# loganmcbroom/Flan

Hardware: AMD Instinct MI355X
Metric: PV analysis+resynthesis frames/sec (2048-win, hop 512, 48 kHz) at 1/2/4/8 GPU (higher is better)
Workload: dtype f32; 1 GPU; 8 ch x 60 s x 48 kHz uniform noise per GPU, convert_to_PV(2048,512,dft 2048) -> convert_to_audio round trip; channels_per_gpu=8, parallelism=channel-shard x1

## Files before the change

flan_amd/csrc/conversions.hip:

```cpp
#include "flanhip_internal.h"
#include <atomic>
#include <memory>
#include "pv_kernels.h"
#include "pv_kernels_fast.h"
#include <type_traits>
#include "pv_kernels_v2.h"
#include "pv_kernels_v3.h"
#include "pv_kernels_eo.h"
#include "pv_kernels_any.h"
#include "pv_kernels_mr.h"
#include "pv_kernels_bs.h"
#include "pv_kernels_big.h"
#include "team_launch.h"
#include "sub_launch.h"
#include <algorithm>
#include <cstdlib>

namespace flanhip {


static constexpr size_t kMaxLds = 160 * 1024;

static constexpr int kMaxAnyDft = 1 << 20;
static bool fft_size( int dft ) { return is_pow2( dft ) && dft >= 32 && dft <= 8192; }
// ... 138 lines not shown
	return size_t( C ) * 8 + size_t( wpad ) * 4 + size_t( chains ) * ( size_t( padded_len( C + 1 ) ) * 8 + size_t( wpad ) * 4 );
	}

template<int LOG2C, int WAVES, int T = 1>
static int run_analyze( const AnalyzeParams & p, hipStream_t s )
	{
	const size_t lds = analyze_lds_bytes( 1 << LOG2C, p.window_size, WAVES, LOG2C >= 12 && T == 1 );
	FLANHIP_REQUIRE( lds <= kMaxLds, FLANHIP_ERR_UNSUPPORTED, "window/dft too large for LDS" );
	auto kern = k_analyze<LOG2C, WAVES, T>;
	FLANHIP_CHECK( hipFuncSetAttribute( reinterpret_cast<const void*>( kern ), hipFuncAttributeMaxDynamicSharedMemorySize, int( lds ) ) );
	const int64_t chains = int64_t( p.chains_per_channel ) * p.num_channels;
	const int64_t blocks = ( chains + WAVES - 1 ) / WAVES;
	FLANHIP_REQUIRE( blocks < ( int64_t( 1 ) << 31 ), FLANHIP_ERR_UNSUPPORTED, "too many chains for one launch" );
	hipLaunchKernelGGL( kern, dim3( (unsigned) blocks ), dim3( 64 * WAVES * T ), lds, s, p );
	FLANHIP_CHECK( hipGetLastError() );
	return FLANHIP_OK;
	}

#define FLANHIP_V3_CFGS_9( X ) X( 0, 8, 4, 4, 1 )
#define FLANHIP_V3_CFGS_8( X ) X( 0, 4, 3, 4, 1 )
struct V3Cfg { int waves, occ, nv; };
static V3Cfg v3_cfg( int dft )
	{
	const int v = debug_options().ana_variant;
#define X( I, W, O, N, P ) if( v == I ) return V3Cfg{ W, O, N };
	if( dft == 1024 ) { FLANHIP_V3_CFGS_9( X ) return V3Cfg{ 8, 4, 4 }; }
	FLANHIP_V3_CFGS_8( X )
#undef X
	return V3Cfg{ 4, 3, 4 };
	}
static int v3_index( int dft )
	{
	const int v = debug_options().ana_variant;
#define X( I, W, O, N, P ) if( v == I ) return I;
	if( dft == 1024 ) { FLANHIP_V3_CFGS_9( X ) return 0; }
	FLANHIP_V3_CFGS_8( X )
#undef X
	return 0;
	}
static bool v3_size( int dft ) { return dft == 1024 || dft == 512; }
static int group_size_of( int dft ) { return dft == 2048 ? 8 : dft == 4096 ? 4 : v3_size( dft ) ? v3_cfg( dft ).waves : 8; }
static constexpr int kTeamWaves12 = 8;
static int generic_target_chains( int dft ) { const int cus = cu_count(); return dft >= 8192 ? cus : dft == 4096 ? 2 * cus : dft == 2048 ? 4 * cus : 16 * cus; }
static int fast_target_chains( int dft, bool synth )
	{
	if( const int v = debug_options().target_chains ) { if( v > 0 ) return v; }
	return cu_count() * ( dft == 4096 ? 4 : dft == 2048 ? 8 : 4 * v3_cfg( dft ).occ );
	}

template<int WAVES, bool SUMS, int NV, int ABL = 0>
static int run_analyze_v2( const AnalyzeParams & p, const FastTables & tb, hipStream_t s )
	{
	FLANHIP_REQUIRE( ( int64_t( WAVES ) * p.L + 2 ) * std::max( int64_t( p.hop ) * 4, int64_t( 8200 ) ) < ( int64_t( 1 ) << 32 ), FLANHIP_ERR_UNSUPPORTED, "chain length x hop too large for the dft 2048 kernel" );
	const size_t lds = V2Lds::bytes( WAVES );
	static_assert( V2Lds::bytes( WAVES ) <= kMaxLds, "LDS budget" );
	auto kern = k_analyze_v2<WAVES, SUMS, NV, ABL>;
	FLANHIP_CHECK( hipFuncSetAttribute( reinterpret_cast<const void*>( kern ), hipFuncAttributeMaxDynamicSharedMemorySize, int( lds ) ) );
	const int64_t blocks = int64_t( ( p.chains_per_channel + WAVES - 1 ) / WAVES ) * p.num_channels;
	FLANHIP_REQUIRE( blocks < ( int64_t( 1 ) << 31 ), FLANHIP_ERR_UNSUPPORTED, "too many chains for one launch" );
	hipLaunchKernelGGL( kern, dim3( (unsigned) blocks ), dim3( 64 * WAVES ), lds, s, p, tb );
	FLANHIP_CHECK( hipGetLastError() );
	return FLANHIP_OK;
	}

template<bool SUMS>
static int run_analyze_v2_variant( int v, const AnalyzeParams & p, const FastTables & tb, hipStream_t s )
	{
	switch( v )
		{
		default: return run_analyze_v2<8, SUMS, 8>( p, tb, s );
#ifdef FLANHIP_ABLATIONS
		case 101: return run_analyze_v2<8, SUMS, 8, 1>( p, tb, s );
		case 102: return run_analyze_v2<8, SUMS, 8, 2>( p, tb, s );
		case 104: return run_analyze_v2<8, SUMS, 8, 4>( p, tb, s );
		case 108: return run_analyze_v2<8, SUMS, 8, 8>( p, tb, s );
		case 116: return run_analyze_v2<8, SUMS, 8, 16>( p, tb, s );
		case 132: return run_analyze_v2<8, SUMS, 8, 32>( p, tb, s );
		case 106: return run_analyze_v2<8, SUMS, 8, 6>( p, tb, s );
		case 124: return run_analyze_v2<8, SUMS, 8, 24>( p, tb, s );
		case 163: return run_analyze_v2<8, SUMS, 8, 63>( p, tb, s );
		case 164: return run_analyze_v2<8, SUMS, 8, 64>( p, tb, s );
		case 228: return run_analyze_v2<8, SUMS, 8, 128>( p, tb, s );
		case 292: return run_analyze_v2<8, SUMS, 8, 192>( p, tb, s );
		case 139: return run_analyze_v2<8, SUMS, 8, 39>( p, tb, s );
		case 107: return run_analyze_v2<8, SUMS, 8, 7>( p, tb, s );
		case 356: return run_analyze_v2<8, SUMS, 8, 256>( p, tb, s );
		case 1124: return run_analyze_v2<8, SUMS, 8, 1024>( p, tb, s );
		case 1163: return run_analyze_v2<8, SUMS, 8, 1024 + 39>( p, tb, s );
		case 612: return run_analyze_v2<8, SUMS, 8, 512>( p, tb, s );
		case 868: return run_analyze_v2<8, SUMS, 8, 768>( p, tb, s );
#endif
		}
	}

template<int LOG2C, bool SUMS, int WAVES, int OCC, int NV, int PF>
static int run_analyze_v3( const AnalyzeParams & p, hipStream_t s )
	{
	using L = V3Lds<LOG2C>;
	FLANHIP_REQUIRE( ( int64_t( WAVES ) * p.L + 2 ) * std::max( int64_t( p.hop ) * 4, int64_t( ( L::C + 1 ) * 8 ) ) < ( int64_t( 1 ) << 32 ), FLANHIP_ERR_UNSUPPORTED, "chain length x hop too large for the dft 1024 / 512 kernel" );
	const size_t lds = L::bytes( WAVES, true );
	static_assert( L::bytes( WAVES, true ) * ( 4 * OCC / WAVES ) <= kMaxLds, "LDS budget" );
	auto kern = k_analyze_v3<LOG2C, WAVES, SUMS, OCC, NV, ( PF & 255 ), ( PF >> 8 )>;
	FLANHIP_CHECK( hipFuncSetAttribute( reinterpret_cast<const void*>( kern ), hipFuncAttributeMaxDynamicSharedMemorySize, int( lds ) ) );
	const int64_t blocks = int64_t( ( p.chains_per_channel + WAVES - 1 ) / WAVES ) * p.num_channels;
	FLANHIP_REQUIRE( blocks < ( int64_t( 1 ) << 31 ), FLANHIP_ERR_UNSUPPORTED, "too many chains for one launch" );
	hipLaunchKernelGGL( kern, dim3( (unsigned) blocks ), dim3( 64 * WAVES ), lds, s, p );
	FLANHIP_CHECK( hipGetLastError() );
	return FLANHIP_OK;
	}
template<bool SUMS>
static int run_analyze_v3_cfg( int dft, const AnalyzeParams & p, hipStream_t s )
	{
	const int idx = v3_index( dft );
#define X( I, W, O, N, P ) if( idx == I ) return run_analyze_v3<9, SUMS, W, O, N, P>( p, s );
	if( dft == 1024 ) { FLANHIP_V3_CFGS_9( X ) }
#undef X
#define X( I, W, O, N, P ) if( idx == I ) return run_analyze_v3<8, SUMS, W, O, N, P>( p, s );
	if( dft == 512 ) { FLANHIP_V3_CFGS_8( X ) }
#undef X
	return FLANHIP_ERR_UNSUPPORTED;
// ... 707 lines not shown

int flanhip_synthesize_dev_fused_checked( const flanhip_MF * d_pv, int64_t ch, int64_t F, int bins, float sr, float ar, int W,
	float * d_out, void * d_ws, int * d_nan, void * stream )
	{
	return launch_synthesize( d_pv, ch, F, bins, sr, ar, W, d_out, d_ws, d_nan, 2, (hipStream_t) stream );
	}

int flanhip_analyze( const float * audio, int64_t ch, int64_t n, float sr, int W, int hop, int dft,
	flanhip_MF * out, int64_t * num_pv_frames, volatile int * cancel )
	{
	FLANHIP_REQUIRE( audio && out, FLANHIP_ERR_INVALID_ARG, "null buffer" );
	FLANHIP_REQUIRE( ch > 0 && n >= 0 && hop >= 1, FLANHIP_ERR_INVALID_ARG, "bad sizes" );
	if( int rc = require_device() ) return rc;
	const int64_t F = n / hop + 1;
	const int bins = dft / 2 + 1;
	if( num_pv_frames ) *num_pv_frames = F;
	if( cancelled( cancel ) ) return FLANHIP_ERR_CANCELLED;
	DeviceBuffer d_audio, d_pv;
	if( int rc = d_audio.alloc( sizeof( float ) * size_t( ch ) * n ) ) return rc;
	if( int rc = d_pv.alloc( sizeof( flanhip_MF ) * size_t( ch ) * F * bins ) ) return rc;
	if( int rc_t = flanhip_upload( d_audio.p, audio, sizeof( float ) * size_t( ch ) * n ) ) return rc_t;
	if( cancelled( cancel ) ) return FLANHIP_ERR_CANCELLED;
	if( int rc = launch_analyze( (const float*) d_audio.p, ch, n, sr, W, hop, dft, (flanhip_MF*) d_pv.p, nullptr, nullptr ) ) return rc;
	if( int rc = wait_cancellable( nullptr, cancel ? poll_volatile_int : nullptr, const_cast<int*>( cancel ) ) ) return rc;
	if( int rc_t = flanhip_download( out, d_pv.p, sizeof( flanhip_MF ) * size_t( ch ) * F * bins ) ) return rc_t;
	return FLANHIP_OK;
	}

int flanhip_synthesize_dev_stages( const flanhip_MF * d_pv, int64_t ch, int64_t F, int bins, float sr, float ar, int W,
	float * d_out, void * d_ws, int * d_nan, int presummed, int stages, void * stream )
	{
	FLANHIP_REQUIRE( presummed >= 0 && presummed <= 2, FLANHIP_ERR_INVALID_ARG, "presummed: 0, 1 or 2" );
	return launch_synthesize( d_pv, ch, F, bins, sr, ar, W, d_out, d_ws, d_nan, presummed, (hipStream_t) stream, nullptr, nullptr, false, stages );
	}

void flanhip_debug_option( int which, int value )
	{
	DebugOptions & o = debug_options();
	switch( which )
		{
		case FLANHIP_DEBUG_CHAIN_LEN:       o.chain_len = value; break;
		case FLANHIP_DEBUG_TARGET_CHAINS:   o.target_chains = value; break;
		case FLANHIP_DEBUG_FORCE_GENERIC:   o.force_generic = value; break;
		case FLANHIP_DEBUG_NO_FAST_DIV:     o.no_fast_div = value; break;
		case FLANHIP_DEBUG_ANA_VARIANT:     o.ana_variant = value; break;
		case FLANHIP_DEBUG_SYN_VARIANT:     o.syn_variant = value; break;
		case FLANHIP_DEBUG_ANA4096_OLD:     o.ana11_old = value; break;
		case FLANHIP_DEBUG_SYN4096_OLD:     o.syn11_old = value; break;
		case FLANHIP_DEBUG_RESAMPLE_DIRECT: o.resample_direct = value; break;
		case FLANHIP_DEBUG_FORCE_DIRECT:    o.force_direct = value; break;
		case FLANHIP_DEBUG_INLINE_FIXUP:    o.inline_fixup = value; break;
		case FLANHIP_DEBUG_WIDE_OFFSETS:    o.wide_offsets = value; break;
		case FLANHIP_DEBUG_NO_SUB:          o.no_sub = value; break;
		default: break;
		}
	}
#ifdef FLANHIP_STAMPS
int flanhip_debug_read_stamps( unsigned long long * out16 )
	{
	FLANHIP_CHECK( hipDeviceSynchronize() );
	FLANHIP_CHECK( hipMemcpyFromSymbol( out16, HIP_SYMBOL( g_stamp_acc ), 16 * sizeof( unsigned long long ) ) );
	unsigned long long zero[16] = { 0 };
	FLANHIP_CHECK( hipMemcpyToSymbol( HIP_SYMBOL( g_stamp_acc ), zero, sizeof( zero ) ) );
	return FLANHIP_OK;
	}
int flanhip_debug_read_spans( unsigned long long * out8192 )
	{
	FLANHIP_CHECK( hipDeviceSynchronize() );
	FLANHIP_CHECK( hipMemcpyFromSymbol( out8192, HIP_SYMBOL( g_stamp_span ), 8192 * sizeof( unsigned long long ) ) );
	return FLANHIP_OK;
	}
#endif

size_t flanhip_synthesize_workspace_bytes( int64_t ch, int64_t F, int bins, float sr, float ar, int W )
	{
	SynthLayout lay;
	if( synth_layout( ch, F, bins, sr, ar, W, &lay ) ) return 0;
	size_t bytes = lay.total_bytes;
	if( v3_size( lay.dft ) )
		{
		DebugOptions & o = debug_options();
		const int keep = o.ana_variant;
		for( int v = 0; v < 3; ++v )
			{
			o.ana_variant = v;
			SynthLayout alt;
			if( !synth_layout( ch, F, bins, sr, ar, W, &alt ) ) bytes = std::max( bytes, alt.total_bytes );
			}
		o.ana_variant = keep;
		}
	return bytes;
	}

int flanhip_synthesize_dev( const flanhip_MF * d_pv, int64_t ch, int64_t F, int bins, float sr, float ar, int W,
	float * d_out, void * d_ws, int * d_nan, void * stream )
	{
	return launch_synthesize( d_pv, ch, F, bins, sr, ar, W, d_out, d_ws, d_nan, false, (hipStream_t) stream );
	}

int flanhip_synthesize( const flanhip_MF * pv, int64_t ch, int64_t F, int bins, float sr, float ar, int W,
	float * out, int * nan_flag, volatile int * cancel )
	{
	FLANHIP_REQUIRE( pv && out, FLANHIP_ERR_INVALID_ARG, "null buffer" );
	SynthLayout lay;
	if( int rc = synth_layout( ch, F, bins, sr, ar, W, &lay ) ) return rc;
	if( int rc = require_device() ) return rc;
// ... 22 lines not shown
```

flan_amd/csrc/flanhip_internal.h:

```cpp
#pragma once
#include <hip/hip_runtime.h>
#include <cstdarg>
#include <cstdint>
#include <cstdio>
#include <cmath>
#include <map>
#include <memory>
#include <mutex>
#include <tuple>
#include <vector>

#include "flanhip.h"
#include "cf_type.h"

namespace flanhip {

void set_error( const char * fmt, ... );

#define FLANHIP_CHECK( expr )                                                                         \
	do { hipError_t e_ = ( expr );                                                                    \
		if( e_ != hipSuccess ) {                                                                      \
			::flanhip::set_error( "%s failed: %s (%s:%d)", #expr, hipGetErrorString( e_ ), __FILE__, __LINE__ ); \
			return FLANHIP_ERR_HIP; } } while( 0 )

#define FLANHIP_REQUIRE( cond, code, msg )                                                            \
	do { if( !( cond ) ) { ::flanhip::set_error( "%s: %s", __func__, msg ); return code; } } while( 0 )

int require_device();

inline bool is_pow2( int64_t n ) { return n > 0 && ( n & ( n - 1 ) ) == 0; }
inline int ilog2( int64_t n ) { int l = 0; while( ( int64_t( 1 ) << l ) < n ) ++l; return l; }
inline bool cancelled( volatile int * c ) { return c && *c != 0; }
int * thread_cancel_word( hipStream_t s );
int wait_cancellable( hipStream_t s, int ( *poll )( void * ), void * user );
inline int poll_volatile_int( void * user ) { volatile int * c = static_cast<volatile int*>( user ); return c && *c != 0; }

struct Plan
	{
	float * d_window = nullptr;
	cf * d_tw = nullptr;
	cf * d_tw2 = nullptr;
	cf * d_tw1f = nullptr;
	cf * d_tw3f = nullptr;
	cf * d_bs_tw = nullptr;
	d2 * d_bs_chirp = nullptr;
	d2 * d_bs_bh = nullptr;
	float * d_dump = nullptr;
	cf * d_team = nullptr;
	};
inline int team_radix( int dft_size ) { return dft_size == 8192 ? 4 : dft_size == 16384 ? 8 : 0; }
struct TeamTableLayout { int tw1, tw3, twj, tws, two, total; };
inline TeamTableLayout team_table_layout( int R ) { TeamTableLayout l; l.tw1 = 0; l.tw3 = 240; l.twj = 1008; l.tws = l.twj + ( R - 1 ) * 512; l.two = l.tws + ( R / 2 ) * 512; l.total = l.two + 2 * R; return l; }
struct PlanRef { Plan plan; PlanRef() = default; PlanRef( const PlanRef & ) = delete; PlanRef & operator=( const PlanRef & ) = delete; ~PlanRef(); };
int get_plan( int window_size, int dft_size, std::shared_ptr<const PlanRef> * out );

struct DivPlan { float c, rc; int exact; };
int get_div_plan( float c, DivPlan * out );

int choose_chain_length( int64_t num_channels, int64_t num_frames, int min_len, int target_chains, int group = 1 );
struct DebugOptions
	{
	int chain_len = 0;
	int target_chains = 0;
	int force_generic = 0;
	int no_fast_div = 0;
	int ana_variant = 0, syn_variant = 0;
	int ana11_old = 0, syn11_old = 0;
	int resample_direct = 0;
	int wide_offsets = 0;
	int inline_fixup = 0;
	int no_sub = 0;
	int force_direct = 0;
	};
DebugOptions & debug_options();
bool force_generic();
int cu_count();

int launch_analyze( const float * d_audio, int64_t ch, int64_t n, float sr, int W, int hop, int dft, flanhip_MF * d_out, void * d_fused_ws, hipStream_t s );
int launch_synthesize( const flanhip_MF * d_pv, int64_t ch, int64_t F, int bins, float sr, float ar, int W, float * d_out,
	void * d_ws, int * d_nan, int presummed, hipStream_t s, const double * d_carry_in = nullptr, double * d_total_out = nullptr,
	bool prepass_only = false, int stage_mask = 0xF );

int next_epoch();

struct SynthLayout { int hop, dft, L, chains_per_channel, head_len, groups_per_channel; size_t carry_bytes, head_bytes, group_offset, group_bytes, total_bytes;
	size_t flags_offset;
	size_t fix_offset, tail_offset;
	bool any; size_t any_spec_offset, any_frames_offset;
	size_t mr_ring_offset;
	size_t bsg_offset;
	bool big; size_t big_out_offset, big_head_offset, big_ring_offset; };
void note_workspace_producer( const void * d_ws, int kind, int epoch = 0 );
int workspace_producer( const void * d_ws, int * epoch = nullptr );
int synth_layout( int64_t ch, int64_t F, int bins, float sr, float ar, int W, SynthLayout * out );

bool valid_interp( int kind );
float interp_eval_host( int kind, float x );
int processors_set_interp_lut( int slot, const float * d_table );
int processors_ext_set_interp_lut( int slot, const float * d_table );
int processors_arrange_set_interp_lut( int slot, const float * d_table );

}
```

flan_amd/csrc/pv_kernels_v2.h:

```cpp
#pragma once
#include "pv_kernels_fast.h"

namespace flanhip {

struct V2Lds
	{
	static constexpr int C = 1024;
	static constexpr int TW1 = 0;
	static constexpr int TW3 = TW1 + 240;
	static constexpr int W2H = TW3 + 768;
	static constexpr int WIN = W2H + 512;
	static constexpr int KC = WIN + 1024;
	static constexpr int BUF = KC + 1024;
	static constexpr int BUF_LEN = C + C / 16 + 1;
	static constexpr size_t bytes( int waves ) { return size_t( BUF + waves * BUF_LEN ) * 8; }
	};


#ifdef FLANHIP_STAMPS
__device__ unsigned long long g_stamp_acc[16];
__device__ unsigned long long g_stamp_span[2 * 4096];
struct Stamps
	{
	unsigned long long last, acc[12], t_begin, r_begin;
	__device__ __forceinline__ static unsigned long long realtime()
		{
		unsigned long long t;
		asm volatile( "s_memrealtime %0\n\ts_waitcnt lgkmcnt(0)" : "=s"( t ) :: "memory" );
		return t;
		}
	__device__ __forceinline__ static unsigned long long now()
		{
		unsigned long long t;
		__builtin_amdgcn_sched_barrier( 0 );
		asm volatile( "s_memtime %0\n\ts_waitcnt lgkmcnt(0)" : "=s"( t ) :: "memory" );
		__builtin_amdgcn_sched_barrier( 0 );
		return t;
		}
#ifdef FLANHIP_STAMPS_CLOCK_ONLY
	__device__ __forceinline__ void init()
		{
		const unsigned long long r = realtime();
		const unsigned w = blockIdx.x * ( blockDim.x >> 6 ) + ( threadIdx.x >> 6 );
		if( ( threadIdx.x & 63 ) == 0 && w < 4096 ) g_stamp_span[2 * w] = r;
		}
#else
	__device__ __forceinline__ void init() { for( int i = 0; i < 12; ++i ) acc[i] = 0; r_begin = realtime(); last = now(); t_begin = last; }
#endif
#ifdef FLANHIP_STAMPS_CLOCK_ONLY
	__device__ __forceinline__ void operator()( int ) const {}
#else
	__device__ __forceinline__ void operator()( int i ) { const unsigned long long t = now(); acc[i] += t - last; last = t; }
#endif
#ifdef FLANHIP_STAMPS_CLOCK_ONLY
	__device__ __forceinline__ void flush( int lane )
		{
		const unsigned long long r = realtime();
		const unsigned w = blockIdx.x * ( blockDim.x >> 6 ) + ( threadIdx.x >> 6 );
		if( lane == 0 && w < 4096 ) { g_stamp_span[2 * w + 1] = r; atomicAdd( &g_stamp_acc[15], 1ull ); }
		}
#else
	__device__ __forceinline__ void flush( int lane )
		{
		const unsigned long long t_end = now(), r_end = realtime();
		if( lane == 0 )
			{
			for( int i = 0; i < 12; ++i ) atomicAdd( &g_stamp_acc[i], acc[i] );
			atomicAdd( &g_stamp_acc[12], t_end - t_begin );
			atomicAdd( &g_stamp_acc[13], r_end - r_begin );
			atomicAdd( &g_stamp_acc[15], 1ull );
			const unsigned w = blockIdx.x * ( blockDim.x >> 6 ) + ( threadIdx.x >> 6 );
			if( w < 4096 ) { g_stamp_span[2 * w] = r_begin; g_stamp_span[2 * w + 1] = r_end; }
			}
		}
#endif
	};
#else
struct Stamps
	{
	__device__ __forceinline__ void init() {}
	__device__ __forceinline__ void operator()( int ) const {}
	__device__ __forceinline__ void flush( int ) {}
	};
#endif


#ifndef FLANHIP_PUBLISH_DRAIN
#define FLANHIP_PUBLISH_DRAIN 1
#endif
__device__ __forceinline__ void publish_drain()
	{
	if constexpr( FLANHIP_PUBLISH_DRAIN != 0 ) asm volatile( "s_waitcnt vmcnt(0)" ::: "memory" );
	else asm volatile( "" ::: "memory" );
	}

template<int WAVES, bool SUMS, int NV, int ABL = 0>
__global__ __launch_bounds__( 64 * WAVES ) void k_analyze_v2( AnalyzeParams p, FastTables tb )
	{
	using L = V2Lds;
	constexpr int C = 1024, E = 16, H = 8, NT = 64 * WAVES;
	constexpr int NP = NV / 2;
	static_assert( NV == 2 || NV == 4 || NV == 8 || NV == 16, "1, 2, 4 or 8 pairs at a time" );
	typedef float VB __attribute__(( ext_vector_type( NV ) ));
	extern __shared__ __attribute__((aligned(16))) unsigned char smem[];
	cf * s = reinterpret_cast<cf*>( smem );
	const int tid = threadIdx.x, lane = tid & 63, wave = tid >> 6;
	const int W = p.window_size, hop = p.hop;
	const int cancel_word = cancel_peek( p.cancel );

	for( int i = tid; i < 240; i += NT ) s[L::TW1 + i] = tb.tw1[i];
	for( int i = tid; i < 768; i += NT ) s[L::TW3 + i] = tb.tw3[i];
	for( int i = tid; i < 512; i += NT ) { const cf w = tb.w2[i]; s[L::W2H + i] = mk( 0.5f * w.x, 0.5f * w.y ); }
		{
		float * win = reinterpret_cast<float*>( s + L::WIN );
		for( int i = tid; i < 2 * C; i += NT ) win[i] = ( i < W ) ? p.window[i] : 0.0f;
		v4f_t * kc = reinterpret_cast<v4f_t*>( s + L::KC );
		const float rdft = 1.0f / float( 2 * C );
		for( int k = tid; k < 512; k += NT )
			{
			const float bk = float( k ) * p.sample_rate * rdft, bm = float( C - k ) * p.sample_rate * rdft;
			kc[k] = v4f_t{ bk, div_c( bk, p.ar_div ) * FLANHIP_PI2_F, bm, div_c( bm, p.ar_div ) * FLANHIP_PI2_F };
			}
		}
	__syncthreads();
	const cf * s_tw1 = s + L::TW1;
	const cf * s_tw3 = s + L::TW3;
	const cf * s_w2 = s + L::W2H + lane;
	const cf * s_win = s + L::WIN + lane;
	const v4f_t * s_kc = reinterpret_cast<const v4f_t*>( s + L::KC ) + lane;
	cf * buf = s + L::BUF + wave * L::BUF_LEN;
	const int groups = ( p.chains_per_channel + WAVES - 1 ) / WAVES;
	const int channel = int( blockIdx.x ) / groups, group = int( blockIdx.x ) % groups;
	const int chain_in_channel = group * WAVES + wave;
	const bool active = chain_in_channel < p.chains_per_channel && !cancel_seen( cancel_word );
	const int64_t chain = int64_t( channel ) * p.chains_per_channel + ( active ? chain_in_channel : 0 );
	const int t0 = ( active ? chain_in_channel : 0 ) * p.L;
	const int t1 = int( min( int64_t( t0 ) + p.L, p.F ) );
	const float * x = p.audio + int64_t( channel ) * p.n;
	const int n32 = int( p.n );
	const int tb0 = group * WAVES * p.L - 1;
	const char * const xb = reinterpret_cast<const char*>( x ) + ( int64_t( hop ) * tb0 - W / 2 ) * 4;
	char * const rb = reinterpret_cast<char*>( p.out + ( int64_t( channel ) * p.F + tb0 ) * ( C + 1 ) );
	const unsigned lane8 = 8u * unsigned( lane );
	const bool use_wrapping = p.analysis_rate < p.sample_rate;
	const float k_ar = p.analysis_rate;
	const DivC k_ard = p.ar_div;
	const int padl = lane + ( lane >> 4 );
	const cf * mirror = buf + ( C * 17 ) / 16 - ( lane + ( ( lane + 15 ) >> 4 ) );
	struct __attribute__(( packed, aligned( 4 ) )) f2u { float x, y; };

	float prevk[H], prevm[H], prevx = 0.0f;
	#pragma unroll
	for( int q = 0; q < H; ++q ) { prevk[q] = 0.0f; prevm[q] = 0.0f; }
	double sumk[SUMS ? H : 1], summ[SUMS ? H : 1], sumx = 0.0;
	if constexpr( SUMS )
		{
		#pragma unroll
		for( int q = 0; q < H; ++q ) { sumk[q] = 0.0; summ[q] = 0.0; }
		}
	unsigned mmax = 0u;
	cf ring = mk( 0.0f, 0.0f );

	const int tfirst = t0 > 0 ? t0 - 1 : t0;
	const bool w_whole = ( W & 127 ) == 0;
	auto frame_inside = [&]( int t ) { return w_whole && hop * t - W / 2 >= 0 && hop * t - W / 2 + 2 * C <= n32; };

	Stamps st;
	st.init();
	cf z[E];
	auto run_chain = [&]()
		{
		auto load_pair = [&]( int t, int q, auto fast_tag ) -> cf
			{
			constexpr bool FAST = decltype( fast_tag )::value;
			const int start = hop * ( ( ABL & 512 ) ? tfirst : t ) - W / 2;
			if constexpr( ( ABL & 16 ) != 0 ) return mk( float( start ) * 1e-9f + 0.25f, float( q ) );
			else if constexpr( ( ABL & 128 ) != 0 && FAST )
				{
				struct __attribute__(( packed, aligned( 4 ) )) f4u { float x, y, z, w; };
				const f4u v = *reinterpret_cast<const f4u*>( x + start + 4 * lane + 256 * ( q / 2 ) );
				return ( q & 1 ) ? mk( v.z, v.w ) : mk( v.x, v.y );
				}
			else if constexpr( FAST )
				{
				const unsigned off = unsigned( hop * ( ( ( ABL & 512 ) ? tfirst : t ) - tb0 ) ) * 4u + lane8 + ( q >= 8 ? 4096u : 0u );
				const f2u v = *reinterpret_cast<const f2u*>( xb + off + 512 * ( q & 7 ) );
				return mk( v.x, v.y );
				}
			else
				{
				const int a0c = min( max( start + 2 * ( lane + 64 * q ), 0 ), n32 - 2 );
				const f2u v = *reinterpret_cast<const f2u*>( x + a0c );
				return mk( v.x, v.y );
				}
			};
		auto fix_raw = [&]( int t )
			{
			const int start = hop * t - W / 2;
			#pragma unroll
			for( int q = 0; q < E; ++q )
				{
				const int s0 = 2 * ( lane + 64 * q );
				const int a0 = start + s0;
				const int d = a0 - min( max( a0, 0 ), n32 - 2 );
				float v0 = ( d == 0 ) ? z[q].x : ( d == 1 ? z[q].y : 0.0f );
				float v1 = ( d == 0 ) ? z[q].y : ( d == -1 ? z[q].x : 0.0f );
				if( s0 >= W ) v0 = 0.0f;
				if( s0 + 1 >= W ) v1 = 0.0f;
				z[q] = mk( v0, v1 );
				}
			};
		auto transform_frame = [&]( int t, auto fast_tag )
			{
			if constexpr( !decltype( fast_tag )::value ) fix_raw( t );
			#pragma unroll
			for( int q = 0; q < E; ++q )
				{
				const cf w = s_win[64 * q];
				z[q] = mk( z[q].x * w.x, z[q].y * w.y );
				}
			st( 0 );
			if constexpr( ( ABL & 1 ) == 0 )
			fft_fast<10>( z, buf, s_tw1, s_tw3, lane, st );
			st( 3 );
			#pragma unroll
			for( int q = H; q < E; ++q ) buf[padl + 68 * q] = z[q];
			wave_sync();
			};

		auto bins_of_frame = [&]( int t, int tn, int fi, auto halo_tag, auto next_fast )
			{
			constexpr bool halo = decltype( halo_tag )::value;
			const cf z512 = buf[544];
			const cf z0 = z[0];
			#pragma unroll
			for( int q = H; q < E; ++q ) z[q] = load_pair( tn, q, next_fast );
			st( 4 );
			const unsigned roff = unsigned( ( ( ABL & 256 ) ? t0 : t ) - tb0 ) * unsigned( ( C + 1 ) * 8 );
			cf * row = reinterpret_cast<cf*>( rb + roff );
			cf * rowk = reinterpret_cast<cf*>( rb + ( roff + lane8 ) );
			cf * rowm = reinterpret_cast<cf*>( rb + ( roff + unsigned( C * 8 ) - lane8 ) );
			cf outk[halo ? 1 : H], outm[halo ? 1 : H];
			#pragma unroll
			for( int g = 0; g < H / NP; ++g )
				{
				VB re, im, pv, binf, expd;
				#pragma unroll
				for( int i = 0; i < NP; ++i )
					{
					const int q = g * NP + i;
					const cf zk = z[q];
					const cf zm = ( ABL & 32 ) ? zk : mirror[-68 * q];
					const cf w = s_w2[64 * q];
					const v4f_t kc = s_kc[64 * q];
					z[q] = load_pair( tn, q, next_fast );
					const float sx = zk.x + zm.x, dy = zk.y + zm.y, dx = zk.x - zm.x, sy = zk.y - zm.y;
					const float t1v = __builtin_fmaf( w.x, dy, w.y * dx );
					const float t2v = __builtin_fmaf( w.x, dx, -( w.y * dy ) );
					float rk = __builtin_fmaf( 0.5f, sx, t1v ), ik = __builtin_fmaf( 0.5f, sy, -t2v );
					float rm = __builtin_fmaf( 0.5f, sx, -t1v ), imv = __builtin_fmaf( -0.5f, sy, -t2v );
					if( q == 0 )
						{
						rk = ( lane == 0 ) ? z0.x + z0.y : rk;  ik = ( lane == 0 ) ? 0.0f : ik;
						rm = ( lane == 0 ) ? z0.x - z0.y : rm;  imv = ( lane == 0 ) ? 0.0f : imv;
						}
					re[i] = rk; im[i] = ik; re[NP + i] = rm; im[NP + i] = imv;
					pv[i] = prevk[q]; pv[NP + i] = prevm[q];
					binf[i] = kc.x; expd[i] = kc.y; binf[NP + i] = kc.z; expd[NP + i] = kc.w;
					}
				VB phase, m;
				if constexpr( ( ABL & 2 ) == 0 ) polar_v( re, im, phase, m ); else { phase = re; m = im; }
				#pragma unroll
				for( int i = 0; i < NP; ++i ) { prevk[g * NP + i] = phase[i]; prevm[g * NP + i] = phase[NP + i]; }
				if constexpr( !halo )
					{
					VB f;
					if constexpr( ( ABL & 4 ) == 0 )
						{
						const VB phase_diff = phase - pv;
						const VB delta_phase = phase_diff - expd;
						VB wrapped = delta_phase;
						if( use_wrapping ) wrapped = delta_phase - vsplat<VB>( FLANHIP_PI2_F ) * round_half_away_v( div_pi2_v( delta_phase ) );
						VB war;
						#pragma unroll
						for( int i = 0; i < NV; ++i ) war[i] = wrapped[i] * k_ar;
						f = binf + div_pi2_v( war );
						}
					else f = phase - pv + binf * expd;
					#pragma unroll
					for( int i = 0; i < NP; ++i )
						{
						const int q = g * NP + i;
						outk[q] = cf{ m[i], f[i] };
						outm[q] = cf{ m[NP + i], f[NP + i] };
						}
					if constexpr( SUMS )
						{
						const VB term = div_c_each( f, k_ard ) * vsplat<VB>( FLANHIP_PI2_F );
						#pragma unroll
						for( int i = 0; i < NP; ++i )
							{
							sumk[g * NP + i] += double( term[i] );
							summ[g * NP + i] += double( term[NP + i] );
							}
						#pragma unroll
						for( int i = 0; i < NV; i += 2 ) mmax = max( mmax, max( __float_as_uint( m[i] ), __float_as_uint( m[i + 1] ) ) );
						}
					}
				st( 5 + ( g & 3 ) );
				}
			if constexpr( !halo )
				{
				#pragma unroll
				for( int q = 0; q < H; ++q )
					{
					if constexpr( ( ABL & 64 ) != 0 )
						{
						if( ( q & 1 ) == 0 )
							{
							*reinterpret_cast<v4f_t*>( reinterpret_cast<float*>( row ) + 4 * ( lane + 64 * ( q / 2 ) ) ) = v4f_t{ outk[q].x, outk[q].y, outk[q + 1].x, outk[q + 1].y };
							*reinterpret_cast<v4f_t*>( reinterpret_cast<float*>( row ) + 4 * ( lane + 64 * ( q / 2 + 4 ) ) ) = v4f_t{ outm[q].x, outm[q].y, outm[q + 1].x, outm[q + 1].y };
							}
						}
					else if constexpr( ( ABL & 1024 ) != 0 )
						{
						rowk[64 * q] = outk[q];
						rowm[-64 * q] = outm[q];
						}
					else if constexpr( ( ABL & 8 ) == 0 )
						{
						__builtin_nontemporal_store( outk[q], rowk + 64 * q );
						__builtin_nontemporal_store( outm[q], rowm - 64 * q );
						}
					else asm volatile( "" :: "v"( outk[q].x ), "v"( outk[q].y ), "v"( outm[q].x ), "v"( outm[q].y ) );
					}
				}
			ring = ( lane == ( fi & 63 ) ) ? z512 : ring;
			wave_sync();
			st( 9 );
			};

		auto flush_half_bin = [&]( int tb, int nb )
			{
			const int t = tb + lane;
			const bool valid = lane < nb && t >= t0;
			const float re = ring.x, im = -ring.y;
			const float phase = atan2_fast( im, re );
			float pvx = __shfl_up( phase, 1 );
			pvx = ( lane == 0 ) ? prevx : pvx;
			prevx = __shfl( phase, nb - 1 );
			const float bx = float( C / 2 ) * p.sample_rate * ( 1.0f / float( 2 * C ) );
			const float phase_diff = phase - pvx;
			const float delta_phase = phase_diff - div_c( bx, p.ar_div ) * FLANHIP_PI2_F;
			const float wrapped = use_wrapping ? delta_phase - FLANHIP_PI2_F * round_half_away( div_pi2( delta_phase ) ) : delta_phase;
			const float f = bx + div_pi2( wrapped * p.analysis_rate );
			const float m = magnitude_scaled( re, im );
			if constexpr( ( ABL & 8 ) == 0 )
				{
				if( valid ) __builtin_nontemporal_store( mk( m, f ), reinterpret_cast<cf*>( rb + ( unsigned( ( ( ABL & 256 ) ? t0 : t ) - tb0 ) * unsigned( ( C + 1 ) * 8 ) + unsigned( C / 2 * 8 ) ) ) );
				}
			else asm volatile( "" :: "v"( m ), "v"( f ) );
			if constexpr( SUMS )
				{
				const float term = div_c( f, p.ar_div ) * FLANHIP_PI2_F;
				const int j0 = __builtin_amdgcn_readfirstlane( ( tb < t0 ) ? 1 : 0 ), j1 = __builtin_amdgcn_readfirstlane( nb );
				for( int j = j0; j < j1; ++j ) sumx += double( __uint_as_float( __builtin_amdgcn_readlane( __float_as_uint( term ), j ) ) );
				mmax = valid ? max( mmax, __float_as_uint( m ) ) : mmax;
				}
			};

		constexpr std::true_type inside{};
		constexpr std::false_type outside{};
		if( frame_inside( tfirst ) )
			{
			#pragma unroll
			for( int q = 0; q < E; ++q ) z[q] = load_pair( tfirst, q, inside );
			transform_frame( tfirst, inside );
			}
		else
			{
			#pragma unroll
			for( int q = 0; q < E; ++q ) z[q] = load_pair( tfirst, q, outside );
			transform_frame( tfirst, outside );
			}
		int fi = 0;
		if( t0 > 0 )
			{
			if( frame_inside( t0 ) ) { bins_of_frame( t0 - 1, t0, fi, std::true_type{}, inside ); transform_frame( t0, inside ); }
			else { bins_of_frame( t0 - 1, t0, fi, std::true_type{}, outside ); transform_frame( t0, outside ); }
			++fi;
			}
		for( int t = t0; t < t1; ++t )
			{
			const int tn = min( t + 1, t1 - 1 );
			const bool more = t + 1 < t1;
			auto rest_of_step = [&]( auto next_fast )
				{
				bins_of_frame( t, tn, fi, std::false_type{}, next_fast );
				++fi;
				if( ( fi & 63 ) == 0 || !more ) flush_half_bin( t + 1 - ( ( ( fi - 1 ) & 63 ) + 1 ), ( ( fi - 1 ) & 63 ) + 1 );
				if( more ) transform_frame( t + 1, next_fast );
				};
			if( frame_inside( tn ) ) rest_of_step( inside ); else rest_of_step( outside );
			}
		};
	if( active ) run_chain();
	st.flush( lane );

	if constexpr( SUMS )
		{
		double * stage = reinterpret_cast<double*>( buf );
		bool bad = mmax >= 0x7f800000u;
		auto fold = [&]( double sq ) -> double
			{
			bad |= !( __builtin_fabs( sq ) <= 1.7976931348623157e308 );
			return ( __builtin_fabs( sq ) < FLANHIP_FOLD_FAST_LIMIT ) ? fold_phase_fast( sq ) : fold_phase_any( sq );
			};
		if( active )
			{
			double * dst = p.sums + chain * ( C + 1 );
			#pragma unroll
			for( int q = 0; q < H; ++q )
				{
				const double a = fold( sumk[q] ), b = fold( summ[q] );
				dst[lane + 64 * q] = a;             stage[lane + 64 * q] = a;
				dst[C - lane - 64 * q] = b;         stage[C - lane - 64 * q] = b;
				}
			const double vx = fold( sumx );
			if( lane == 0 ) { dst[C / 2] = vx; stage[C / 2] = vx; }
			}
		const bool any_bad = __any( bad );
		if( p.nan_out && lane == 0 && active )
			{
			if( chain == 0 ) { p.nan_out[2] = p.nan_epoch; p.nan_out[4] = p.nan_epoch; }
			if( any_bad ) p.nan_out[0] = p.nan_epoch;
			}
		if( p.group_sums )
			{
			__syncthreads();
			const int live = min( WAVES, p.chains_per_channel - group * WAVES );
			double * gdst = p.group_sums + ( int64_t( channel ) * groups + group ) * ( C + 1 );
			for( int bin = tid; bin <= C; bin += NT )
				{
				double run = 0.0;
				for( int w = 0; w < live; ++w )
					{
					const double v = run + reinterpret_cast<const double*>( s + L::BUF + w * L::BUF_LEN )[bin];
					run = ( __builtin_fabs( v ) < FLANHIP_FOLD_FAST_LIMIT ) ? fold_phase_fast( v ) : fold_phase_any( v );
					}
				gdst[bin] = run;
				}
			}
		}
	}

__device__ __forceinline__ void st_agent( cf * p, cf v )
	{
	unsigned long long bits; __builtin_memcpy( &bits, &v, 8 );
	__hip_atomic_store( reinterpret_cast<unsigned long long*>( p ), bits, __ATOMIC_RELAXED, __HIP_MEMORY_SCOPE_AGENT );
	}
__device__ __forceinline__ cf ld_agent( const cf * p )
	{
	const unsigned long long bits = __hip_atomic_load( reinterpret_cast<const unsigned long long*>( p ), __ATOMIC_RELAXED, __HIP_MEMORY_SCOPE_AGENT );
	cf v; __builtin_memcpy( &v, &bits, 8 );
	return v;
	}

struct V2LdsSyn
	{
	static constexpr int C = 1024;
// ... 467 lines not shown
```

include/flanhip.h:

```cpp
#ifndef FLANHIP_H
#define FLANHIP_H

#include <stddef.h>
#include <stdint.h>

#ifdef __cplusplus
extern "C" {
#endif

#define FLANHIP_OK                 0
#define FLANHIP_ERR_INVALID_ARG   -1
#define FLANHIP_ERR_UNSUPPORTED   -2
#define FLANHIP_ERR_HIP           -3
#define FLANHIP_ERR_CANCELLED     -4
#define FLANHIP_ERR_NO_DEVICE     -5

typedef struct flanhip_MF { float m; float f; } flanhip_MF;

int          flanhip_version(void);
const char * flanhip_last_error(void);
int          flanhip_device_count(void);
int          flanhip_set_device(int device);
int          flanhip_get_device(int * device);

// ... 12 lines not shown
int flanhip_upload(void * d_dst, const void * src, size_t bytes);
int flanhip_download(void * dst, const void * d_src, size_t bytes);
int flanhip_touch_pages(void * ptr, size_t bytes);
int flanhip_host_workers(void);
int flanhip_parallel_for(int n_tasks, void (*fn)(void *, int), void * ctx);
int flanhip_stream_create(void ** stream);
int flanhip_stream_destroy(void * stream);
int flanhip_host_malloc(void ** hptr, size_t bytes);
int flanhip_host_free(void * hptr);

int flanhip_analyze(const float * audio, int64_t num_channels, int64_t num_audio_frames, float sample_rate,
                    int window_size, int hop, int dft_size,
                    flanhip_MF * out, int64_t * num_pv_frames, volatile int * cancel);
int flanhip_analyze_dev(const float * d_audio, int64_t num_channels, int64_t num_audio_frames, float sample_rate,
                        int window_size, int hop, int dft_size,
                        flanhip_MF * d_out, void * stream);

int flanhip_synthesize(const flanhip_MF * pv, int64_t num_channels, int64_t num_pv_frames, int num_bins,
                       float sample_rate, float analysis_rate, int window_size,
                       float * out, int * nan_flag, volatile int * cancel);
size_t flanhip_synthesize_workspace_bytes(int64_t num_channels, int64_t num_pv_frames, int num_bins,
                                          float sample_rate, float analysis_rate, int window_size);
int flanhip_synthesize_dev(const flanhip_MF * d_pv, int64_t num_channels, int64_t num_pv_frames, int num_bins,
                           float sample_rate, float analysis_rate, int window_size,
                           float * d_out, void * d_workspace, int * d_nan_flag, void * stream);

int flanhip_analyze_dev_fused(const float * d_audio, int64_t num_channels, int64_t num_audio_frames, float sample_rate,
                              int window_size, int hop, int dft_size,
                              flanhip_MF * d_out, void * d_synth_workspace, void * stream);
int flanhip_synthesize_dev_fused(const flanhip_MF * d_pv, int64_t num_channels, int64_t num_pv_frames, int num_bins,
                                 float sample_rate, float analysis_rate, int window_size,
                                 float * d_out, void * d_workspace, int * d_nan_flag, void * stream);
int flanhip_synthesize_dev_fused_checked(const flanhip_MF * d_pv, int64_t num_channels, int64_t num_pv_frames, int num_bins,
                                         float sample_rate, float analysis_rate, int window_size,
                                         float * d_out, void * d_workspace, int * d_nan_flag, void * stream);

int flanhip_synthesize_dev_stages(const flanhip_MF * d_pv, int64_t num_channels, int64_t num_pv_frames, int num_bins,
                                  float sample_rate, float analysis_rate, int window_size,
                                  float * d_out, void * d_workspace, int * d_nan_flag, int presummed, int stages, void * stream);

#define FLANHIP_DEBUG_CHAIN_LEN       0
#define FLANHIP_DEBUG_TARGET_CHAINS   1
#define FLANHIP_DEBUG_FORCE_GENERIC   2
#define FLANHIP_DEBUG_NO_FAST_DIV     3
#define FLANHIP_DEBUG_ANA_VARIANT     4
#define FLANHIP_DEBUG_SYN_VARIANT     5
#define FLANHIP_DEBUG_ANA4096_OLD     6
#define FLANHIP_DEBUG_SYN4096_OLD     7
#define FLANHIP_DEBUG_RESAMPLE_DIRECT 8
#define FLANHIP_DEBUG_FORCE_DIRECT    9
#define FLANHIP_DEBUG_INLINE_FIXUP   10
#define FLANHIP_DEBUG_WIDE_OFFSETS   11
#define FLANHIP_DEBUG_NO_SUB         12
void flanhip_debug_option(int which, int value);
int flanhip_debug_kernel_scratch_bytes(int which);

int flanhip_modify_time(const flanhip_MF * pv, int64_t num_channels, int64_t num_pv_frames, int num_bins,
                        float sample_rate, int hop, const float * mod_seconds,
                        int64_t out_frames, flanhip_MF * out, volatile int * cancel);
int flanhip_modify_time_dev(const flanhip_MF * d_pv, int64_t num_channels, int64_t num_pv_frames, int num_bins,
                            float sample_rate, int hop, const float * d_mod_seconds,
                            int64_t out_frames, flanhip_MF * d_out, void * stream);
int flanhip_modify_time_dev_fused(const flanhip_MF * d_pv, int64_t num_channels, int64_t num_pv_frames, int num_bins,
                                  float sample_rate, float analysis_rate, const float * d_mod, int64_t out_frames,
                                  flanhip_MF * d_out, int window_size, void * d_workspace, void * stream);
int flanhip_stretch_map_dev(float * d_factor, int64_t num_pv_frames, int num_bins, float sample_rate, int hop,
                            float * d_max, void * stream);
int flanhip_stretch_map_const_dev(float factor, float * d_map, int64_t num_pv_frames, int num_bins, float sample_rate, int hop,
                                  float * d_max, void * stream);
int flanhip_fill_dev(float * d_grid, int64_t count, float value, void * stream);

int flanhip_modify_frequency(const flanhip_MF * pv, int64_t num_channels, int64_t num_pv_frames, int num_bins,
                             float sample_rate, const float * mod_hz, const float * in_modified,
                             flanhip_MF * out, volatile int * cancel);
int flanhip_modify_frequency_dev(const flanhip_MF * d_pv, int64_t num_channels, int64_t num_pv_frames, int num_bins,
                                 float sample_rate, const float * d_mod_hz, const float * d_in_modified,
                                 flanhip_MF * d_out, void * stream);
int flanhip_repitch_map_dev(const flanhip_MF * d_pv, int64_t num_channels, int64_t num_pv_frames, int num_bins,
                            float sample_rate, float * d_factor, float * d_in_modified, void * stream);
int flanhip_repitch_dev(const flanhip_MF * d_pv, int64_t num_channels, int64_t num_pv_frames, int num_bins, float sample_rate,
                        float * d_factor, flanhip_MF * d_out, void * stream);
int flanhip_modify_time_interp_dev(const flanhip_MF * d_pv, int64_t num_channels, int64_t num_pv_frames, int num_bins,
                                   float sample_rate, int hop, const float * d_mod_seconds,
                                   int64_t out_frames, int interp, flanhip_MF * d_out, void * stream);
int flanhip_modify_time_interp_dev_fused(const flanhip_MF * d_pv, int64_t num_channels, int64_t num_pv_frames, int num_bins,
                                         float sample_rate, float analysis_rate, const float * d_mod_seconds,
                                         int64_t out_frames, int interp, flanhip_MF * d_out, int window_size, void * d_synth_workspace, void * stream);
int flanhip_modify_frequency_interp_dev(const flanhip_MF * d_pv, int64_t num_channels, int64_t num_pv_frames, int num_bins,
                                        float sample_rate, const float * d_mod_hz, const float * d_in_modified,
                                        int interp, flanhip_MF * d_out, void * stream);
int flanhip_repitch_interp_dev(const flanhip_MF * d_pv, int64_t num_channels, int64_t num_pv_frames, int num_bins, float sample_rate,
                               float * d_factor, int interp, flanhip_MF * d_out, void * stream);


int flanhip_shape_affine(const flanhip_MF * pv, int64_t num_channels, int64_t num_pv_frames, int num_bins,
                         float sample_rate, float a, float b, float c, float d, int use_shift_alignment,
                         flanhip_MF * out, volatile int * cancel);
int flanhip_shape_affine_dev(const flanhip_MF * d_pv, int64_t num_channels, int64_t num_pv_frames, int num_bins,
                             float sample_rate, float a, float b, float c, float d, int use_shift_alignment,
                             flanhip_MF * d_out, void * stream);
int flanhip_shape_table_dev(const flanhip_MF * d_pv, const flanhip_MF * d_shaped, int64_t num_channels,
                            int64_t num_pv_frames, int num_bins, float sample_rate, int use_shift_alignment,
                            flanhip_MF * d_out, void * stream);
int flanhip_shape_affine_dev_fused(const flanhip_MF * d_pv, int64_t num_channels, int64_t num_frames, int num_bins, float sample_rate,
                                   float analysis_rate, float a, float b, float c, float d, flanhip_MF * d_out, int window_size,
                                   void * d_ws, void * stream);
// ... 123 lines not shown
```

Measured before the change: 168.6 million frames/s.

## Hand off first-frame phases between adjacent waves instead of recomputing halo frame

In the dft-2048 analysis kernel, each wave used to recompute the FFT of the frame just before its chain (a halo) to get the previous phases. Now every wave except the first skips that halo. It writes the raw phase and magnitude of its own first frame into an LDS stash and raises a flag; the previous wave spins on that flag, then finishes the boundary row and accumulates the partial sums. This saves one FFT per chain, at the cost of extra LDS, a spin-wait dependency between waves, an extra __syncthreads, and added code complexity.

```diff
diff --git a/flan_amd/csrc/conversions.hip b/flan_amd/csrc/conversions.hip
--- a/flan_amd/csrc/conversions.hip
+++ b/flan_amd/csrc/conversions.hip
@@ -214,8 +214,9 @@
 static int run_analyze_v2( const AnalyzeParams & p, const FastTables & tb, hipStream_t s )
 	{
 	FLANHIP_REQUIRE( ( int64_t( WAVES ) * p.L + 2 ) * std::max( int64_t( p.hop ) * 4, int64_t( 8200 ) ) < ( int64_t( 1 ) << 32 ), FLANHIP_ERR_UNSUPPORTED, "chain length x hop too large for the dft 2048 kernel" );
-	const size_t lds = V2Lds::bytes( WAVES );
-	static_assert( V2Lds::bytes( WAVES ) <= kMaxLds, "LDS budget" );
+	constexpr bool handoff = ( ABL & 2048 ) == 0;
+	const size_t lds = V2Lds::bytes( WAVES, handoff );
+	static_assert( V2Lds::bytes( WAVES, handoff ) <= kMaxLds, "LDS budget" );
 	auto kern = k_analyze_v2<WAVES, SUMS, NV, ABL>;
 	FLANHIP_CHECK( hipFuncSetAttribute( reinterpret_cast<const void*>( kern ), hipFuncAttributeMaxDynamicSharedMemorySize, int( lds ) ) );
 	const int64_t blocks = int64_t( ( p.chains_per_channel + WAVES - 1 ) / WAVES ) * p.num_channels;
@@ -228,6 +229,7 @@
 template<bool SUMS>
 static int run_analyze_v2_variant( int v, const AnalyzeParams & p, const FastTables & tb, hipStream_t s )
 	{
+	if( debug_options().ana2048_halo ) return run_analyze_v2<8, SUMS, 8, 2048>( p, tb, s );
 	switch( v )
 		{
 		default: return run_analyze_v2<8, SUMS, 8>( p, tb, s );
@@ -1041,6 +1043,7 @@
 		case FLANHIP_DEBUG_INLINE_FIXUP:    o.inline_fixup = value; break;
 		case FLANHIP_DEBUG_WIDE_OFFSETS:    o.wide_offsets = value; break;
 		case FLANHIP_DEBUG_NO_SUB:          o.no_sub = value; break;
+		case FLANHIP_DEBUG_ANA2048_HALO:    o.ana2048_halo = value; break;
 		default: break;
 		}
 	}
diff --git a/flan_amd/csrc/flanhip_internal.h b/flan_amd/csrc/flanhip_internal.h
--- a/flan_amd/csrc/flanhip_internal.h
+++ b/flan_amd/csrc/flanhip_internal.h
@@ -70,6 +70,7 @@
 	int wide_offsets = 0;
 	int inline_fixup = 0;
 	int no_sub = 0;
+	int ana2048_halo = 0;
 	int force_direct = 0;
 	};
 DebugOptions & debug_options();
diff --git a/flan_amd/csrc/pv_kernels_v2.h b/flan_amd/csrc/pv_kernels_v2.h
--- a/flan_amd/csrc/pv_kernels_v2.h
+++ b/flan_amd/csrc/pv_kernels_v2.h
@@ -13,7 +13,10 @@
 	static constexpr int KC = WIN + 1024;
 	static constexpr int BUF = KC + 1024;
 	static constexpr int BUF_LEN = C + C / 16 + 1;
-	static constexpr size_t bytes( int waves ) { return size_t( BUF + waves * BUF_LEN ) * 8; }
+	static constexpr int STASH_LEN = C + 1;
+	static constexpr int stash( int waves ) { return BUF + waves * BUF_LEN; }
+	static constexpr int flags( int waves ) { return stash( waves ) + ( waves - 1 ) * STASH_LEN; }
+	static constexpr size_t bytes( int waves, bool handoff = false ) { return size_t( handoff ? flags( waves ) + waves / 2 + 1 : BUF + waves * BUF_LEN ) * 8; }
 	};
 
 
@@ -106,7 +109,9 @@
 	cf * s = reinterpret_cast<cf*>( smem );
 	const int tid = threadIdx.x, lane = tid & 63, wave = tid >> 6;
 	const int W = p.window_size, hop = p.hop;
+	constexpr bool HANDOFF = ( ABL & 2048 ) == 0;
 	const int cancel_word = cancel_peek( p.cancel );
+	int * const hflag = reinterpret_cast<int*>( s + L::flags( WAVES ) );
 
 	for( int i = tid; i < 240; i += NT ) s[L::TW1 + i] = tb.tw1[i];
 	for( int i = tid; i < 768; i += NT ) s[L::TW3 + i] = tb.tw3[i];
@@ -121,6 +126,11 @@
 			const float bk = float( k ) * p.sample_rate * rdft, bm = float( C - k ) * p.sample_rate * rdft;
 			kc[k] = v4f_t{ bk, div_c( bk, p.ar_div ) * FLANHIP_PI2_F, bm, div_c( bm, p.ar_div ) * FLANHIP_PI2_F };
 			}
+		}
+	if constexpr( HANDOFF )
+		{
+		if( tid < WAVES ) hflag[tid] = 0;
+		if( tid == 0 ) hflag[WAVES] = cancel_word;
 		}
 	__syncthreads();
 	const cf * s_tw1 = s + L::TW1;
@@ -132,7 +142,13 @@
 	const int groups = ( p.chains_per_channel + WAVES - 1 ) / WAVES;
 	const int channel = int( blockIdx.x ) / groups, group = int( blockIdx.x ) % groups;
 	const int chain_in_channel = group * WAVES + wave;
-	const bool active = chain_in_channel < p.chains_per_channel && !cancel_seen( cancel_word );
+	bool cancelled;
+	if constexpr( HANDOFF ) cancelled = __builtin_amdgcn_readfirstlane( hflag[WAVES] ) != 0;
+	else cancelled = cancel_seen( cancel_word );
+	const bool active = chain_in_channel < p.chains_per_channel && !cancelled;
+	const bool deferred = HANDOFF && __builtin_amdgcn_readfirstlane( int( active && wave > 0 ) ) != 0;
+	const bool consumer = HANDOFF && __builtin_amdgcn_readfirstlane( int( active && wave + 1 < WAVES && chain_in_channel + 1 < p.chains_per_channel ) ) != 0;
+	cf * const stash_own = s + L::stash( WAVES ) + ( deferred ? wave - 1 : 0 ) * L::STASH_LEN;
 	const int64_t chain = int64_t( channel ) * p.chains_per_channel + ( active ? chain_in_channel : 0 );
 	const int t0 = ( active ? chain_in_channel : 0 ) * p.L;
 	const int t1 = int( min( int64_t( t0 ) + p.L, p.F ) );
@@ -161,7 +177,8 @@
 	unsigned mmax = 0u;
 	cf ring = mk( 0.0f, 0.0f );
 
-	const int tfirst = t0 > 0 ? t0 - 1 : t0;
+	const int tfirst = ( t0 > 0 && !deferred ) ? t0 - 1 : t0;
+	const int tstore = deferred ? t0 + 1 : t0;
 	const bool w_whole = ( W & 127 ) == 0;
 	auto frame_inside = [&]( int t ) { return w_whole && hop * t - W / 2 >= 0 && hop * t - W / 2 + 2 * C <= n32; };
 
@@ -228,9 +245,25 @@
 			wave_sync();
 			};
 
-		auto bins_of_frame = [&]( int t, int tn, int fi, auto halo_tag, auto next_fast )
-			{
-			constexpr bool halo = decltype( halo_tag )::value;
+		auto freq_of = [&]( const VB phase, const VB pv, const VB binf, const VB expd ) -> VB
+			{
+			if constexpr( ( ABL & 4 ) == 0 )
+				{
+				const VB phase_diff = phase - pv;
+				const VB delta_phase = phase_diff - expd;
+				VB wrapped = delta_phase;
+				if( use_wrapping ) wrapped = delta_phase - vsplat<VB>( FLANHIP_PI2_F ) * round_half_away_v( div_pi2_v( delta_phase ) );
+				VB war;
+				#pragma unroll
+				for( int i = 0; i < NV; ++i ) war[i] = wrapped[i] * k_ar;
+				return binf + div_pi2_v( war );
+				}
+			else return phase - pv + binf * expd;
+			};
+		auto bins_of_frame = [&]( int t, int tn, int fi, auto mode_tag, auto next_fast )
+			{
+			constexpr int mode = decltype( mode_tag )::value;
+			constexpr bool halo = mode != 0;
 			const cf z512 = buf[544];
 			const cf z0 = z[0];
 			#pragma unroll
@@ -272,21 +305,19 @@
 				if constexpr( ( ABL & 2 ) == 0 ) polar_v( re, im, phase, m ); else { phase = re; m = im; }
 				#pragma unroll
 				for( int i = 0; i < NP; ++i ) { prevk[g * NP + i] = phase[i]; prevm[g * NP + i] = phase[NP + i]; }
+				if constexpr( mode == 2 )
+					{
+					#pragma unroll
+					for( int i = 0; i < NP; ++i )
+						{
+						const int q = g * NP + i;
+						stash_own[lane + 64 * q] = cf{ phase[i], m[i] };
+						stash_own[C - lane - 64 * q] = cf{ phase[NP + i], m[NP + i] };
+						}
+					}
 				if constexpr( !halo )
 					{
-					VB f;
-					if constexpr( ( ABL & 4 ) == 0 )
-						{
-						const VB phase_diff = phase - pv;
-						const VB delta_phase = phase_diff - expd;
-						VB wrapped = delta_phase;
-						if( use_wrapping ) wrapped = delta_phase - vsplat<VB>( FLANHIP_PI2_F ) * round_half_away_v( div_pi2_v( delta_phase ) );
-						VB war;
-						#pragma unroll
-						for( int i = 0; i < NV; ++i ) war[i] = wrapped[i] * k_ar;
-						f = binf + div_pi2_v( war );
-						}
-					else f = phase - pv + binf * expd;
+					const VB f = freq_of( phase, pv, binf, expd );
 					#pragma unroll
 					for( int i = 0; i < NP; ++i )
 						{
@@ -336,25 +367,31 @@
 					}
 				}
 			ring = ( lane == ( fi & 63 ) ) ? z512 : ring;
+			if constexpr( mode == 2 ) { if( lane == 0 ) stash_own[C / 2] = z512; }
 			wave_sync();
 			st( 9 );
 			};
 
+		auto half_bin_mf = [&]( float re, float im, float phase, float pvx ) -> cf
+			{
+			const float bx = float( C / 2 ) * p.sample_rate * ( 1.0f / float( 2 * C ) );
+			const float phase_diff = phase - pvx;
+			const float delta_phase = phase_diff - div_c( bx, p.ar_div ) * FLANHIP_PI2_F;
+			const float wrapped = use_wrapping ? delta_phase - FLANHIP_PI2_F * round_half_away( div_pi2( delta_phase ) ) : delta_phase;
+			const float f = bx + div_pi2( wrapped * p.analysis_rate );
+			return mk( magnitude_scaled( re, im ), f );
+			};
 		auto flush_half_bin = [&]( int tb, int nb )
 			{
 			const int t = tb + lane;
-			const bool valid = lane < nb && t >= t0;
+			const bool valid = lane < nb && t >= tstore;
 			const float re = ring.x, im = -ring.y;
 			const float phase = atan2_fast( im, re );
 			float pvx = __shfl_up( phase, 1 );
 			pvx = ( lane == 0 ) ? prevx : pvx;
 			prevx = __shfl( phase, nb - 1 );
-			const float bx = float( C / 2 ) * p.sample_rate * ( 1.0f / float( 2 * C ) );
-			const float phase_diff = phase - pvx;
-			const float delta_phase = phase_diff - div_c( bx, p.ar_div ) * FLANHIP_PI2_F;
-			const float wrapped = use_wrapping ? delta_phase - FLANHIP_PI2_F * round_half_away( div_pi2( delta_phase ) ) : delta_phase;
-			const float f = bx + div_pi2( wrapped * p.analysis_rate );
-			const float m = magnitude_scaled( re, im );
+			const cf mf = half_bin_mf( re, im, phase, pvx );
+			const float m = mf.x, f = mf.y;
 			if constexpr( ( ABL & 8 ) == 0 )
 				{
 				if( valid ) __builtin_nontemporal_store( mk( m, f ), reinterpret_cast<cf*>( rb + ( unsigned( ( ( ABL & 256 ) ? t0 : t ) - tb0 ) * unsigned( ( C + 1 ) * 8 ) + unsigned( C / 2 * 8 ) ) ) );
@@ -363,7 +400,7 @@
 			if constexpr( SUMS )
 				{
 				const float term = div_c( f, p.ar_div ) * FLANHIP_PI2_F;
-				const int j0 = __builtin_amdgcn_readfirstlane( ( tb < t0 ) ? 1 : 0 ), j1 = __builtin_amdgcn_readfirstlane( nb );
+				const int j0 = __builtin_amdgcn_readfirstlane( ( tb < tstore ) ? 1 : 0 ), j1 = __builtin_amdgcn_readfirstlane( nb );
 				for( int j = j0; j < j1; ++j ) sumx += double( __uint_as_float( __builtin_amdgcn_readlane( __float_as_uint( term ), j ) ) );
 				mmax = valid ? max( mmax, __float_as_uint( m ) ) : mmax;
 				}
@@ -383,25 +420,103 @@
 			for( int q = 0; q < E; ++q ) z[q] = load_pair( tfirst, q, outside );
 			transform_frame( tfirst, outside );
 			}
+		constexpr std::integral_constant<int, 0> a_row{};
+		constexpr std::integral_constant<int, 1> the_halo{};
+		constexpr std::integral_constant<int, 2> handed_over{};
 		int fi = 0;
-		if( t0 > 0 )
-			{
-			if( frame_inside( t0 ) ) { bins_of_frame( t0 - 1, t0, fi, std::true_type{}, inside ); transform_frame( t0, inside ); }
-			else { bins_of_frame( t0 - 1, t0, fi, std::true_type{}, outside ); transform_frame( t0, outside ); }
+		if( tfirst < t0 )
+			{
+			if( frame_inside( t0 ) ) { bins_of_frame( t0 - 1, t0, fi, the_halo, inside ); transform_frame( t0, inside ); }
+			else { bins_of_frame( t0 - 1, t0, fi, the_halo, outside ); transform_frame( t0, outside ); }
 			++fi;
 			}
-		for( int t = t0; t < t1; ++t )
+		auto step = [&]( int t, auto mode_tag )
 			{
 			const int tn = min( t + 1, t1 - 1 );
 			const bool more = t + 1 < t1;
 			auto rest_of_step = [&]( auto next_fast )
 				{
-				bins_of_frame( t, tn, fi, std::false_type{}, next_fast );
+				bins_of_frame( t, tn, fi, mode_tag, next_fast );
 				++fi;
 				if( ( fi & 63 ) == 0 || !more ) flush_half_bin( t + 1 - ( ( ( fi - 1 ) & 63 ) + 1 ), ( ( fi - 1 ) & 63 ) + 1 );
 				if( more ) transform_frame( t + 1, next_fast );
 				};
 			if( frame_inside( tn ) ) rest_of_step( inside ); else rest_of_step( outside );
+			};
+		int t = t0;
+		if constexpr( HANDOFF )
+			{
+			if( deferred )
+				{
+				step( t0, handed_over );
+				if( lane == 0 ) __hip_atomic_store( hflag + wave, 1, __ATOMIC_RELEASE, __HIP_MEMORY_SCOPE_WORKGROUP );
+				t = t0 + 1;
+				}
+			}
+		for( ; t < t1; ++t ) step( t, a_row );
+
+		if constexpr( HANDOFF )
+			{
+			if( consumer )
+				{
+				int spins = 0;
+				while( __builtin_amdgcn_readfirstlane( __hip_atomic_load( hflag + wave + 1, __ATOMIC_ACQUIRE, __HIP_MEMORY_SCOPE_WORKGROUP ) ) == 0 && spins < ( 1 << 20 ) )
+					{
+					__builtin_amdgcn_s_sleep( 32 );
+					++spins;
+					}
+				if( spins >= ( 1 << 20 ) ) mmax = 0xffffffffu;
+				else
+					{
+					cf * const theirs = s + L::stash( WAVES ) + wave * L::STASH_LEN;
+					const unsigned roff = unsigned( t1 - tb0 ) * unsigned( ( C + 1 ) * 8 );
+					cf * rowk = reinterpret_cast<cf*>( rb + ( roff + lane8 ) );
+					cf * rowm = reinterpret_cast<cf*>( rb + ( roff + unsigned( C * 8 ) - lane8 ) );
+					#pragma unroll
+					for( int g = 0; g < H / NP; ++g )
+						{
+						VB phase, m, pv, binf, expd;
+						#pragma unroll
+						for( int i = 0; i < NP; ++i )
+							{
+							const int q = g * NP + i;
+							const cf a = theirs[lane + 64 * q], b = theirs[C - lane - 64 * q];
+							const v4f_t kc = s_kc[64 * q];
+							phase[i] = a.x; m[i] = a.y; phase[NP + i] = b.x; m[NP + i] = b.y;
+							pv[i] = prevk[q]; pv[NP + i] = prevm[q];
+							binf[i] = kc.x; expd[i] = kc.y; binf[NP + i] = kc.z; expd[NP + i] = kc.w;
+							}
+						const VB f = freq_of( phase, pv, binf, expd );
+						VB term;
+						if constexpr( SUMS ) term = div_c_each( f, k_ard ) * vsplat<VB>( FLANHIP_PI2_F );
+						#pragma unroll
+						for( int i = 0; i < NP; ++i )
+							{
+							const int q = g * NP + i;
+							if constexpr( ( ABL & 8 ) == 0 )
+								{
+								__builtin_nontemporal_store( cf{ m[i], f[i] }, rowk + 64 * q );
+								__builtin_nontemporal_store( cf{ m[NP + i], f[NP + i] }, rowm - 64 * q );
+								}
+							if constexpr( SUMS )
+								{
+								theirs[lane + 64 * q].x = term[i];
+								theirs[C - lane - 64 * q].x = term[NP + i];
+								mmax = max( mmax, max( __float_as_uint( m[i] ), __float_as_uint( m[NP + i] ) ) );
+								}
+							}
+						}
+					const cf zx = theirs[C / 2];
+					const float re = zx.x, im = -zx.y;
+					const cf mf = half_bin_mf( re, im, atan2_fast( im, re ), prevx );
+					if( lane == 0 )
+						{
+						if constexpr( ( ABL & 8 ) == 0 ) __builtin_nontemporal_store( mf, reinterpret_cast<cf*>( rb + ( roff + unsigned( C / 2 * 8 ) ) ) );
+						if constexpr( SUMS ) theirs[C / 2].x = div_c( mf.y, p.ar_div ) * FLANHIP_PI2_F;
+						}
+					if constexpr( SUMS ) mmax = max( mmax, __float_as_uint( mf.x ) );
+					}
+				}
 			}
 		};
 	if( active ) run_chain();
@@ -416,6 +531,20 @@
 			bad |= !( __builtin_fabs( sq ) <= 1.7976931348623157e308 );
 			return ( __builtin_fabs( sq ) < FLANHIP_FOLD_FAST_LIMIT ) ? fold_phase_fast( sq ) : fold_phase_any( sq );
 			};
+		if constexpr( HANDOFF )
+			{
+			__syncthreads();
+			if( deferred )
+				{
+				#pragma unroll
+				for( int q = 0; q < H; ++q )
+					{
+					sumk[q] += double( stash_own[lane + 64 * q].x );
+					summ[q] += double( stash_own[C - lane - 64 * q].x );
+					}
+				sumx += double( stash_own[C / 2].x );
+				}
+			}
 		if( active )
 			{
 			double * dst = p.sums + chain * ( C + 1 );
diff --git a/include/flanhip.h b/include/flanhip.h
--- a/include/flanhip.h
+++ b/include/flanhip.h
@@ -88,6 +88,7 @@
 #define FLANHIP_DEBUG_INLINE_FIXUP   10
 #define FLANHIP_DEBUG_WIDE_OFFSETS   11
 #define FLANHIP_DEBUG_NO_SUB         12
+#define FLANHIP_DEBUG_ANA2048_HALO  13
 void flanhip_debug_option(int which, int value);
 int flanhip_debug_kernel_scratch_bytes(int which);
 
```

New measurement: 167.6 million frames/s. No clear change (-0.6%).
